# data61/stellar-random-walk

Measured on AMD Instinct MI355X. Metric: walk-steps/sec, higher is better.
Workload: dtype f64

## Files before the change

### stellar-random-walk_amd/csrc/walk_kernels.hip

```cpp
#include <algorithm>
#include <map>
#include <tuple>
#include <chrono>
#include <cstring>

#include "engine.h"
#include "sampling.h"
#include "walk_records.h"

namespace srw {
namespace {
constexpr int TILE = 16;

__device__ inline const Row *row_of(const GraphView &g, int32_t v) {
  int64_t s = (int64_t)v - g.vmin;
  if (s < 0 || s >= g.n_slots) return nullptr;
  return g.rows + s;
}

__device__ inline void flush_counters(DevCounters *ctr, unsigned long long steps, unsigned long long dead,
                                      unsigned long long degc, unsigned long long degp, unsigned long long reads,
                                      unsigned long long fb) {
  steps = wave_sum_u64(steps); dead = wave_sum_u64(dead); degc = wave_sum_u64(degc);
  degp = wave_sum_u64(degp); reads = wave_sum_u64(reads); fb = wave_sum_u64(fb);
  if (lane_id() == 0) {
    if (steps) atomicAdd(&ctr->steps, steps);
    if (dead) atomicAdd(&ctr->dead_ends, dead);
    if (degc) atomicAdd(&ctr->sum_deg_curr, degc);
    if (degp) atomicAdd(&ctr->sum_deg_prev, degp);
    if (reads) atomicAdd(&ctr->ent_reads, reads);
    if (fb) atomicAdd(&ctr->fallbacks, fb);
  }
}

template <bool NT, int MINW, bool COMPACT>
__global__ __launch_bounds__(TPB, MINW) void k_walk_first_order(GraphView g, const int32_t *__restrict__ verts,
                                                          int64_t n_verts, int64_t n_walkers, int32_t L,
                                                          int32_t first_walk, RngSpec rng,
                                                          int32_t *__restrict__ paths, int32_t *__restrict__ lens,
                                                          DevCounters *ctr) {
  __shared__ int32_t tile[TPB / 64][64][TILE + 1];
  const int lane = lane_id(), wv = threadIdx.x >> 6;
  const int64_t wi = blockIdx.x * (int64_t)TPB + threadIdx.x;
  const int64_t wave_base = wi - lane;
  const int64_t stride = (int64_t)L + 2;
  bool alive = wi < n_walkers;
  uint32_t iter = 0; int32_t src = 0;
  Row r; r.off = 0; r.deg = 0; r.flags = 0;
  if (alive) {
    int64_t it = wi / n_verts, vi = wi - it * n_verts;
    iter = (uint32_t)(first_walk + it);
    src = verts[vi];
    const Row *rp = row_of(g, src);
    if (rp) r = *rp;
  }
  int32_t len = 1;
  unsigned long long reads = 0, dead = 0, fb = 0;
  Bias nobias; nobias.second_order = false; nobias.need_member = false; nobias.p = nobias.q = 1.0f;
  nobias.prev = 0; nobias.prev_sids = nullptr; nobias.prev_deg = 0; nobias.vmin = g.vmin;
  tile[wv][lane][0] = src;
  src = rng_source(g, src);
  for (int32_t s = 1; s <= L + 1; ++s) {
    const int c = s & (TILE - 1);
    int32_t val = -1;
    if (alive) {
      if (r.deg == 0) {
        alive = false; if (s > 1) ++dead;
      } else {
        if (COMPACT && !(r.flags & ROW_IRREGULAR)) {
          const uint32_t m = walk_bits24(rng.seed, iter, (uint32_t)src, (uint32_t)s);
          unsigned rd;
          const CfoEnt e = cfo_pick<NT>(g.cfo + r.off, r.deg, m, rd); reads += rd;
          val = e.id; ++len;
          r.off = (int64_t)(e.link & CFO_NOFF_MASK); r.deg = (int32_t)((e.link >> 40) & 0x7FFFFFu);
          r.flags = (e.link >> 63) ? ROW_IRREGULAR : 0u;
        } else {
          float u = draw_uniform(rng, iter, (uint32_t)src, (uint32_t)s);
          FoEnt e;
          if (r.flags & ROW_IRREGULAR) {
            int32_t k = lane_pick_sequential(g.ent + r.off, r.deg, nobias, u);
            ++fb;
            if (COMPACT) {
              const CfoEnt ce = g.cfo[r.off + k];
              e.id = ce.id; e.noff = (int64_t)(ce.link & CFO_NOFF_MASK); e.ndeg = (int32_t)((ce.link >> 40) & 0x7FFFFFu);
              e.nflags = (ce.link >> 63) ? ROW_IRREGULAR : 0u;
            } else {
              e = g.fo[r.off + k];
            }
          } else {
            unsigned rd; int32_t k;
            e = fo_pick<NT>(g.fo + r.off, r.deg, u, k, rd); reads += rd;
          }
          val = e.id; ++len;
          r.off = e.noff; r.deg = e.ndeg; r.flags = e.nflags;
        }
      }
    }
    tile[wv][lane][c] = val;
    if (c == TILE - 1 || s == L + 1) {
      const int ncols = c + 1;
      const int64_t base_slot = s - c;
      __syncthreads();
#pragma unroll
      for (int rr = 0; rr < 16; ++rr) {
        int row = rr * 4 + (lane >> 4), col = lane & 15;
        int64_t w = wave_base + row;
        if (col < ncols && w < n_walkers) paths[w * stride + base_slot + col] = tile[wv][row][col];
      }
      __syncthreads();
    }
  }
  if (wi < n_walkers) lens[wi] = len;
  flush_counters(ctr, (unsigned long long)(len - 1), dead, 0, 0, reads, fb);
}

__device__ inline Bias make_bias(const GraphView &g, float p, float q, int32_t prev, bool second_order) {
  Bias b;
  b.p = p; b.q = q; b.prev = prev; b.second_order = second_order;
  b.need_member = second_order && (q != 1.0f);
  b.prev_sids = nullptr; b.prev_deg = 0; b.vmin = g.vmin;
  if (b.need_member) {
    int64_t s = (int64_t)prev - g.vmin;
    if (s >= 0 && s < g.n_slots) { Row r = g.mrows[s]; b.prev_sids = g.msids + r.off; b.prev_deg = r.deg; b.prev_hub = r.flags >> ROW_HUB_SHIFT; }
  }
  return b;
}

__global__ __launch_bounds__(TPB, 4) void k_walk_general(GraphView g, const int32_t *__restrict__ verts,
                                                      int64_t n_verts, int64_t n_walkers, int32_t L,
                                                      int32_t first_walk, RngSpec rng, float p, float q,
                                                      int32_t *__restrict__ paths, int32_t *__restrict__ lens,
                                                      DevCounters *ctr, unsigned long long *cursor, int32_t tune,
                                                      const int32_t *__restrict__ todo, const unsigned long long *todo_n,
                                                      const int32_t *__restrict__ todo_tie, const ChainRec *__restrict__ tie_list,
                                                      const SWalker *__restrict__ tie_out) {
  __shared__ __attribute__((aligned(16))) uint32_t bitmap[TPB / 64][BINNED_LDS_WORDS];
  const int lane = lane_id();
  Member mem; mem.mode = 0; mem.bm = bitmap[threadIdx.x >> 6]; mem.seg_base = 0;
  mem.ehash = g.ehash; mem.ehash_mask = g.ehash_mask;
#ifdef SRW_PHASE_TIMING
  const unsigned long long t_begin = wall_clock64();
#endif
  const int64_t stride = (int64_t)L + 2;
  unsigned long long steps = 0, degc = 0, degp = 0, fb = 0, dead = 0, fast = 0, srch = 0;
  unsigned long long n_strat[12] = {0, 0, 0, 0, 0, 0, 0, 0, 0, 0, 0, 0};
  while (true) {
    unsigned long long grab = 0;
    if (lane == 0) grab = atomicAdd(cursor, 1ull);
    int64_t wi = (int64_t)(((unsigned long long)(uint32_t)__builtin_amdgcn_readfirstlane((int)(grab >> 32)) << 32) |
                           (uint32_t)__builtin_amdgcn_readfirstlane((int)(uint32_t)grab));
    int32_t tie_s = -1, tie_k = 0, tie_next = 0;
    if (todo) {
      if (wi >= (int64_t)*todo_n) break;
      if (todo_tie) {
        const int32_t ci = todo_tie[wi];
        if (ci >= 0) {
          const SWalker o = tie_out[ci];
          if (o.kind == SK_WALKER_RET || o.kind == SK_RET) { tie_s = (int32_t)tie_list[ci].pad; tie_k = o.pad0; tie_next = o.curr; }
        }
      }
      wi = todo[wi];
    } else if (wi >= n_walkers) break;
    int64_t it = wi / n_verts, vi = wi - it * n_verts;
    const uint32_t iter = (uint32_t)(first_walk + it);
    const int32_t src = verts[vi];
    const uint32_t ksrc = (uint32_t)rng_source(g, src);
    int32_t *path = paths + wi * stride;
    if (lane == 0) path[0] = src;
    int32_t prev = src, curr = src, len = 1;
    Row rprev; rprev.off = 0; rprev.deg = 0; rprev.flags = 0;
    int64_t eprev = 0;
    for (int32_t s = 1; s <= L + 1; ++s) {
      const bool second = s > 1;
      const int64_t cslot = (int64_t)curr - g.vmin;
      const bool in_range = cslot >= 0 && cslot < g.n_slots;
      const bool want_tab = g.eb_off && second && q != 1.0f && !(tune & 16);
      Row r = g.rows[in_range ? cslot : 0];
      uint32_t eo = EB_NONE;
      if (want_tab) eo = g.eb_off[eprev];
      if (!in_range) { r.off = 0; r.deg = 0; r.flags = 0; }
      if (r.deg == 0) { dead += s > 1; break; }
      Bias b;
      b.p = p; b.q = q; b.prev = prev; b.second_order = second; b.need_member = second && (q != 1.0f); b.vmin = g.vmin;
      b.prev_sids = g.sids + rprev.off; b.prev_deg = rprev.deg; b.prev_hub = rprev.flags >> ROW_HUB_SHIFT;
      float u = draw_uniform(rng, iter, ksrc, (uint32_t)s);
      unsigned f = 0, sv = 0;
#ifdef SRW_PHASE_TIMING
      mem.t_step0 = wall_clock64();
#endif
      SRW_T0(mem);
      int32_t k = -1, next = 0;
      bool binned_served = false, have_next = false;
      unsigned which = SRW_STRAT_SCAN;
      if (s == tie_s) { k = tie_k; next = tie_next; have_next = true; binned_served = true; which = SRW_STRAT_EDGE_TABLE; f = 1; n_strat[SRW_STAT_TIES_RESOLVED] += 1; }
      else if (want_tab) {
        if (r.deg <= g.eb_mask_max) {
          if (r.deg <= 32 || eo != EB_NONE) {
            k = wave_pick_masked(g, r, b, eo, r.deg > 32 ? g.em_bits + (size_t)eo * 4 : nullptr, u, f, next);
            have_next = true; binned_served = true; which = SRW_STRAT_EDGE_MASK;
            srch += 8ull * (unsigned long long)r.deg + 4ull * (unsigned long long)((r.deg + 31) >> 5);
          }
        } else if (eo != EB_NONE && (r.flags & ROW_PQ_OK)) {
          k = wave_pick_edge_table(g, r, b, g.eb_bins + (size_t)eo * 8, u, f, sv, mem, next, mem.bm + 2 * BIN_CAP);
          if (k >= 0) { have_next = true; binned_served = true; which = SRW_STRAT_EDGE_TABLE; srch += 8ull * EB_BINS; }
        }
      }
      if (k < 0 && (!b.need_member || (tune & 16))) {
        k = wave_pick_prefix(g, r, cslot, b, mem.bm, u, f, sv);
        if (k >= 0) which = SRW_STRAT_PREFIX;
      }
      SRW_T1(mem, t_prefix);
      if (k < 0 && !(tune & 16)) {
        unsigned su = 0;
        k = wave_pick_binned(g, r, cslot, b, mem.bm, u, f, sv, tune & 7, (tune & 8) != 0, mem, srch, su, next);
        binned_served = k >= 0;
        if (k >= 0) { have_next = true; which = su == 1 ? SRW_STRAT_P1 : su == 2 ? SRW_STRAT_P2 : su == 4 ? SRW_STRAT_P3 : SRW_STRAT_W; }
      }
      if (k < 0) { k = wave_pick_scan(g, r, b, mem, u, f); degc += (unsigned long long)r.deg; }
      else { fast += sv; }
      n_strat[which] += 1; n_strat[SRW_STRAT_CHAIN] += f;
      if (!have_next) next = g.ent[r.off + k].id;
#ifdef SRW_PHASE_TIMING
      mem.t_strat[which] += wall_clock64() - mem.t_step0 + (unsigned long long)(next & 0);
#endif
      fb += f;
      if (b.need_member && !binned_served) degp += (unsigned long long)b.prev_deg;
      if (lane == 0) path[s] = next;
      prev = curr; curr = next; ++len; rprev = r; eprev = r.off + k;
    }
    for (int64_t t = len + lane; t < stride; t += 64) path[t] = -1;
    if (lane == 0) lens[wi] = len;
    steps += (unsigned long long)(len - 1);
  }
  if (lane == 0) {
    if (steps) atomicAdd(&ctr->steps, steps);
    if (dead) atomicAdd(&ctr->dead_ends, dead);
    if (degc) atomicAdd(&ctr->sum_deg_curr, degc);
    if (degp) atomicAdd(&ctr->sum_deg_prev, degp);
    if (fb) atomicAdd(&ctr->fallbacks, fb);
    if (fast) atomicAdd(&ctr->ent_reads, fast);
    srch += mem.res_bytes;
    if (srch) atomicAdd(&ctr->trials, srch);
    for (int i = 0; i < 12; ++i) if (n_strat[i]) atomicAdd(&ctr->strat[i], n_strat[i]);
#ifdef SRW_PHASE_TIMING
    const unsigned long long tv[10] = {wall_clock64() - t_begin, mem.t_prefix, mem.t_a, mem.t_p1, mem.t_p2, mem.t_w,
                                       mem.t_fin, mem.t_fill, mem.t_pass1, mem.t_pass2};
    for (int i = 0; i < 10; ++i) atomicAdd(&ctr->dbg[i], tv[i] >> 10);
    atomicAdd(&ctr->dbg[10], mem.n_w); atomicAdd(&ctr->dbg[11], mem.n_w_elems); atomicAdd(&ctr->dbg[12], mem.n_w_windows);
    atomicAdd(&ctr->dbg[13], mem.n_p1); atomicAdd(&ctr->dbg[14], mem.n_p1_elems); atomicAdd(&ctr->dbg[15], mem.n_binned);
    for (int i = 0; i < 12; ++i) atomicAdd(&ctr->dbg[24 + i], mem.t_strat[i] >> 10);
    atomicAdd(&ctr->dbg[16], mem.t_w_lb >> 10); atomicAdd(&ctr->dbg[17], mem.t_w_ins >> 10); atomicAdd(&ctr->dbg[18], mem.t_w_la >> 10); atomicAdd(&ctr->dbg[19], mem.t_w_probe >> 10);
#endif
  }
}

#ifndef SRW_LEAN_WAVES
#define SRW_LEAN_WAVES 8
#endif
#ifndef SRW_LEAN_WAVES_BF
#define SRW_LEAN_WAVES_BF 8
#endif
// ... 113 lines not shown
        const unsigned long long t = atomicAdd(ah.todo_n, 1ull);
        ah.todo[t] = (int32_t)wi;
        if (ah.tie.todo_tie) ah.tie.todo_tie[t] = tie_rec;
        atomicAdd(&ah.ctr->strat[SRW_STAT_HANDED_OVER], 1ull);
      }
      continue;
    }
#ifdef SRW_PATH_BUF
    {
      const int64_t b0 = (int64_t)(len & ~63);
      if (b0 + lane < stride) path[b0 + lane] = pbuf;
      for (int64_t t = b0 + 64 + lane; t < stride; t += 64) path[t] = -1;
    }
#else
    for (int64_t t = len + lane; t < stride; t += 64) path[t] = -1;
#endif
    if (lane == 0) TAB_ARGS().lens[wi] = len;
    steps += (unsigned long long)(len - 1); n_first += len > 1 ? 1u : 0u;
    fb += w_fb; dead += w_dead; fast += w_fast; srch += w_srch; n_tab += w_tab; n_mask += w_mask;
  }
  if (lane == 0) {
    DevCounters *ctr = TAB_ARGS().ctr;
    srch += mem.res_bytes;
    if (steps) atomicAdd(&ctr->steps, steps);
    if (dead) atomicAdd(&ctr->dead_ends, (unsigned long long)dead);
    if (fb) { atomicAdd(&ctr->fallbacks, (unsigned long long)fb); atomicAdd(&ctr->strat[SRW_STRAT_CHAIN], (unsigned long long)fb); }
    if (fast) atomicAdd(&ctr->ent_reads, (unsigned long long)fast);
    if (srch) atomicAdd(&ctr->trials, srch);
    if (n_tab) atomicAdd(&ctr->strat[SRW_STRAT_EDGE_TABLE], (unsigned long long)n_tab);
    if (n_mask) atomicAdd(&ctr->strat[SRW_STRAT_EDGE_MASK], (unsigned long long)n_mask);
    if (n_first) atomicAdd(&ctr->strat[SRW_STRAT_SCAN], (unsigned long long)n_first);
#ifdef SRW_PHASE_TIMING
    atomicAdd(&ctr->dbg[1], mem.t_a >> 10); atomicAdd(&ctr->dbg[2], mem.t_p1 >> 10); atomicAdd(&ctr->dbg[3], mem.t_p2 >> 10);
    atomicAdd(&ctr->dbg[10], mem.n_w); atomicAdd(&ctr->dbg[11], mem.n_w_elems); atomicAdd(&ctr->dbg[12], mem.n_w_windows);
    atomicAdd(&ctr->dbg[13], mem.n_p1); atomicAdd(&ctr->dbg[14], mem.n_p1_elems); atomicAdd(&ctr->dbg[15], mem.n_binned);
    atomicAdd(&ctr->dbg[16], mem.t_fin);
#endif
  }
}

template <bool NT>
__device__ inline int q1_pick(const GraphView &g, const Row &r, const CfoEnt *crow, uint32_t rv, int32_t rv_pos0, float rv_w0, int32_t prev_id,
                              uint32_t m, float p, CfoEnt &e, int32_t &k, unsigned long long &reads, double *S_out = nullptr) {
  const PqRow PQ(g, r.off);
  int32_t rp[REV_MAX_RETURNS]; double rc[REV_MAX_RETURNS];
  int nr = 0;
  double corr_all = 0.0;
  int64_t so = 0;
  if (rv != REV_NONE) {
    nr = (int)(rv >> 24);
    so = r.off + (int64_t)(rv & 0xFFFFFFu);
    if (nr >= 255) {
      const uint32_t xprev = (uint32_t)((int64_t)prev_id - g.vmin);
      const int64_t row_end = r.off + r.deg;
      while (so + nr < row_end && g.sids[so + nr] == xprev) ++nr;
    }
#pragma unroll
    for (int i = 0; i < REV_MAX_RETURNS; ++i) {
      rp[i] = r.deg; rc[i] = 0.0;
      if (i < nr) {
        float w;
        if (i == 0) { rp[0] = rv_pos0; w = rv_w0; }
        else { rp[i] = (int32_t)g.sperm[so + i]; w = g.sw[so + i]; }
        rc[i] = (double)div_exact(w, p) - (double)w; corr_all += rc[i];
      }
    }
    for (int i = REV_MAX_RETURNS; i < nr; ++i) { const float w = g.sw[so + i]; corr_all += (double)div_exact(w, p) - (double)w; }
  } else {
#pragma unroll
    for (int i = 0; i < REV_MAX_RETURNS; ++i) { rp[i] = r.deg; rc[i] = 0.0; }
  }
  {
    const double S0 = PQ[r.deg - 1], S = S0 + corr_all;
    const double pS = (double)m * 0x1p-24 * S;
    auto corr_upto = [&](int32_t kk) {
      double a = 0.0;
#pragma unroll
      for (int i = 0; i < REV_MAX_RETURNS; ++i) a += (rp[i] <= kk) ? rc[i] : 0.0;
      for (int i = REV_MAX_RETURNS; i < nr; ++i)
        if ((int32_t)g.sperm[so + i] <= kk) { const float w = g.sw[so + i]; a += (double)div_exact(w, p) - (double)w; }
      return a;
    };
    auto numer = [&](int32_t kk) { return PQ[kk] + corr_upto(kk); };
    auto not_miss = [&](int32_t kk, double num) { return !(num * (1.0 + (double)(kk + 8) * 0x1p-51) < pS); };
    auto guide_start = [&](double tau, bool &ok) {
      double f = tau / S0;
      f = f < 0.0 ? 0.0 : (f > 0.99999994 ? 0.99999994 : f);
      const uint32_t mm = (uint32_t)(f * 16777216.0);
      const uint32_t j = (uint32_t)(((uint64_t)mm * (uint64_t)(uint32_t)r.deg) >> 24);
      const CfoEnt ge = load_cfo<NT>(crow + j); ++reads;
      const int32_t gd = cfo_delta(ge.cg, ge.link);
      if (gd == CFO_GD_SAT) { ok = false; return 0; }
      const int32_t st = (int32_t)j - gd;
      return st < 0 ? 0 : (st >= r.deg ? r.deg - 1 : st);
    };
    bool ok = S > 0.0 && S0 > 0.0;
    int32_t k0 = 0;
    if (ok) {
      k0 = guide_start(pS, ok);
      const double cb = ok ? corr_upto(k0) : 0.0;
      if (ok && cb != 0.0) {
        int32_t first_r = r.deg;
#pragma unroll
        for (int i = 0; i < REV_MAX_RETURNS; ++i) first_r = rp[i] < first_r ? rp[i] : first_r;
        for (int i = REV_MAX_RETURNS; i < nr; ++i) { const int32_t q_ = (int32_t)g.sperm[so + i]; first_r = q_ < first_r ? q_ : first_r; }
        const int32_t k1 = guide_start(pS - cb, ok);
        k0 = k1 < first_r ? first_r : k1;
      }
    }
    const bool usable = S > 0.0 && S0 > 0.0;
    if (!usable) return 1;
    else if (S_out && g.dbg_chain_deg && r.deg >= g.dbg_chain_deg) { *S_out = S; return 2; }
    else {
      int guard = 0;
      double nk = 0.0;
      if (ok) {
        nk = numer(k0);
        bool nm = not_miss(k0, nk);
        while (nm && k0 > 0 && guard < 12) {
          const double np = numer(k0 - 1);
          if (!not_miss(k0 - 1, np)) break;
          --k0; nk = np; ++guard;
        }
        while (!nm && guard < 12) {
          ++k0; ++guard;
          if (k0 >= r.deg) break;
          nk = numer(k0); nm = not_miss(k0, nk);
        }
        reads += (unsigned)guard + 1u;
      }
      if (!ok || guard >= 12) {
        int32_t lo = 0, hi = r.deg;
        while (lo < hi) {
          const int32_t mid = lo + ((hi - lo) >> 1);
          if (not_miss(mid, numer(mid))) hi = mid; else lo = mid + 1;
          ++reads;
        }
        k0 = lo;
        if (k0 < r.deg) nk = numer(k0);
      }
      if (k0 >= r.deg) { k = 0; e = load_cfo<NT>(crow); ++reads; }
      else if (nk * (1.0 - (double)(k0 + 8) * 0x1p-51) >= pS) { k = k0; e = load_cfo<NT>(crow + k); ++reads; }
      else { if (S_out) *S_out = S; return 2; }
    }
  }
  return 0;
}

template <bool NT>
__global__ __launch_bounds__(TPB) void k_walk_q1(GraphView g, const int32_t *__restrict__ verts, int64_t n_verts,
                                                 int64_t n_walkers, int32_t L, int32_t first_walk, RngSpec rng, float p,
                                                 int32_t *__restrict__ paths, int32_t *__restrict__ lens, DevCounters *ctr,
                                                 int32_t *__restrict__ todo, unsigned long long *todo_n, uint32_t max_ret) {
  __shared__ int32_t tile[TPB / 64][64][TILE + 1];
  const int lane = lane_id(), wv = threadIdx.x >> 6;
  const int64_t wi = blockIdx.x * (int64_t)TPB + threadIdx.x;
  const int64_t wave_base = wi - lane;
  const int64_t stride = (int64_t)L + 2;
  bool alive = wi < n_walkers, handed = false;
  uint32_t iter = 0; int32_t src = 0;
  Row r; r.off = 0; r.deg = 0; r.flags = 0;
  if (alive) {
    const int64_t it = wi / n_verts, vi = wi - it * n_verts;
    iter = (uint32_t)(first_walk + it);
    src = verts[vi];
    const Row *rp = row_of(g, src);
    if (rp) r = *rp;
  }
  int32_t len = 1;
  int64_t eprev = 0;
  int32_t prev_id = src, curr_id = src;
  unsigned long long reads = 0, dead = 0;
  tile[wv][lane][0] = src;
  src = rng_source(g, src);
  for (int32_t s = 1; s <= L + 1; ++s) {
    const int c = s & (TILE - 1);
    int32_t val = -1;
    bool big = false; uint32_t big_rv = 0u, big_m = 0u;
    if (alive) {
      if (r.deg == 0) {
        alive = false; if (s > 1) ++dead;
      } else if (r.flags & ROW_IRREGULAR) {
        alive = false; handed = true; atomicAdd(&ctr->why[0], 1ull);
      } else {
        const uint32_t m = walk_bits24(rng.seed, iter, (uint32_t)src, (uint32_t)s);
        const CfoEnt *crow = g.cfo + r.off;
        CfoEnt e; int32_t k = -1;
        if (s == 1) {
          unsigned rd; e = cfo_pick<NT>(crow, r.deg, m, rd, k); reads += rd;
        } else {
          const int4v rv4 = NT ? __builtin_nontemporal_load(reinterpret_cast<const int4v *>(g.rev + eprev))
                               : *reinterpret_cast<const int4v *>(g.rev + eprev);
          if ((uint32_t)rv4.x != REV_NONE && ((uint32_t)rv4.x >> 24) > max_ret) { big = true; big_rv = (uint32_t)rv4.x; big_m = m; }
          else {
            const int why = q1_pick<NT>(g, r, crow, (uint32_t)rv4.x, rv4.y, __int_as_float(rv4.z), prev_id, m, p, e, k, reads);
            if (why) { alive = false; handed = true; atomicAdd(&ctr->why[why], 1ull); }
          }
        }
        if (alive && !big) {
          val = e.id; ++len;
          prev_id = curr_id; curr_id = val;
          eprev = r.off + k;
          r.off = (int64_t)(e.link & CFO_NOFF_MASK); r.deg = (int32_t)((e.link >> 40) & 0x7FFFFFu);
          r.flags = (e.link >> 63) ? ROW_IRREGULAR : 0u;
        }
      }
    }
    unsigned long long mb = __ballot(big);
    while (mb) {
      const int l = __ffsll((long long)mb) - 1;
      mb &= mb - 1ull;
      Row rr;
      rr.off = (int64_t)(((unsigned long long)(uint32_t)__builtin_amdgcn_readlane((int)(uint32_t)((uint64_t)r.off >> 32), l) << 32) |
                         (uint32_t)__builtin_amdgcn_readlane((int)(uint32_t)r.off, l));
      rr.deg = __builtin_amdgcn_readlane(r.deg, l); rr.flags = ROW_PQ_OK;
      const int32_t pv = __builtin_amdgcn_readlane(prev_id, l);
      const uint32_t rvl = (uint32_t)__builtin_amdgcn_readlane((int)big_rv, l);
      const uint32_t ml = (uint32_t)__builtin_amdgcn_readlane((int)big_m, l);
      const int64_t so = rr.off + (int64_t)(rvl & 0xFFFFFFu);
      int32_t nr = (int32_t)(rvl >> 24);
      if (nr >= 255) {
        const uint32_t xprev = (uint32_t)((int64_t)pv - g.vmin);
        nr = 0;
        for (int64_t cc = so;; cc += 64) {
          const unsigned long long mm = __ballot(cc + lane < rr.off + rr.deg && g.sids[cc + lane] == xprev);
          nr += __popcll(mm);
          if (mm != ~0ull) break;
        }
      }
      Bias b; b.p = p; b.q = 1.0f; b.prev = pv; b.second_order = true; b.need_member = false; b.vmin = g.vmin;
      b.prev_sids = nullptr; b.prev_deg = 0; b.prev_hub = 0;
      unsigned f = 0;
      const int32_t kk = wave_pick_returns<false>(g, rr, b, so, nr, (float)ml * (1.0f / 16777216.0f), f);
      if (lane == l) {
        big = false;
        if (kk < 0) { alive = false; handed = true; atomicAdd(&ctr->why[kk == CHAIN_NEEDED ? 2 : 1], 1ull); }
        else {
          const CfoEnt e = load_cfo<NT>(g.cfo + r.off + kk); ++reads;
          val = e.id; ++len;
          prev_id = curr_id; curr_id = val;
          eprev = r.off + kk;
          r.off = (int64_t)(e.link & CFO_NOFF_MASK); r.deg = (int32_t)((e.link >> 40) & 0x7FFFFFu);
          r.flags = (e.link >> 63) ? ROW_IRREGULAR : 0u;
        }
      }
    }
    tile[wv][lane][c] = val;
    if (c == TILE - 1 || s == L + 1) {
      const int ncols = c + 1;
      const int64_t base_slot = s - c;
      __syncthreads();
#pragma unroll
      for (int rr = 0; rr < 16; ++rr) {
        int row = rr * 4 + (lane >> 4), col = lane & 15;
        int64_t w = wave_base + row;
        if (col < ncols && w < n_walkers) paths[w * stride + base_slot + col] = tile[wv][row][col];
      }
      __syncthreads();
    }
  }
  if (wi < n_walkers) {
    if (handed) { todo[atomicAdd(todo_n, 1ull)] = (int32_t)wi; atomicAdd(&ctr->strat[SRW_STAT_HANDED_OVER], 1ull); }
    else lens[wi] = len;
  }
  const unsigned long long my_steps = handed ? 0ull : (unsigned long long)(len - 1);
  flush_counters(ctr, my_steps, handed ? 0ull : dead, 0, 0, reads, 0);
  const unsigned long long tot = wave_sum_u64(my_steps);
  if (lane == 0 && tot) atomicAdd(&ctr->strat[SRW_STRAT_Q1_LANE], tot);
}

template <bool NT>
__device__ inline AEnt load_al_head(const AEnt *p) {
  const int4v *q = reinterpret_cast<const int4v *>(p);
  const int4v a = NT ? __builtin_nontemporal_load(q) : *q;
  AEnt e;
  e.prob = __int_as_float(a.x); e.alias = a.y; e.id = a.z; e.wrev = __int_as_float(a.w);
  e.noff = 0; e.ndeg = 0; e.nflags = 0;
  return e;
}
template <bool NT>
__device__ inline void load_al_tail(const AEnt *p, AEnt &e) {
  const int4v *q = reinterpret_cast<const int4v *>(p) + 1;
  const int4v b = NT ? __builtin_nontemporal_load(q) : *q;
  e.noff = (int64_t)(((uint64_t)(uint32_t)b.y << 32) | (uint32_t)b.x);
  e.ndeg = b.z; e.nflags = (uint32_t)b.w;
}

template <bool NT>
__global__ __launch_bounds__(TPB, 6) void k_walk_alias(GraphView g, const int32_t *__restrict__ verts, int64_t n_verts,
                                                    int64_t n_walkers, int32_t L, int32_t first_walk, uint32_t seed,
                                                    float p, float q, int32_t *__restrict__ paths,
                                                    int32_t *__restrict__ lens, DevCounters *ctr) {
  __shared__ int32_t stage[TPB][TILE + 1];
  int32_t *buf = stage[threadIdx.x];
  const int64_t wi = blockIdx.x * (int64_t)TPB + threadIdx.x;
  unsigned long long reads = 0, dead = 0, fb = 0, trials = 0;
  int32_t len = 0;
  if (wi < n_walkers) {
    const int64_t stride = (int64_t)L + 2;
    const int64_t it = wi / n_verts, vi = wi - it * n_verts;
    const uint32_t iter = (uint32_t)(first_walk + it);
    const int32_t src = verts[vi];
    const uint32_t ksrc = (uint32_t)rng_source(g, src);
    int32_t *path = paths + wi * stride;
    Row rc; rc.off = 0; rc.deg = 0; rc.flags = 0;
    { const Row *rp0 = row_of(g, src); if (rp0) rc = *rp0; }
    Row rp = rc;
    int32_t curr = src, prev = src;
    buf[0] = src; len = 1;
    const float inv_p = 1.0f / p, inv_q = 1.0f / q;
    const float Q = inv_q > 1.0f ? inv_q : 1.0f;
    const bool biased_cfg = !(p == 1.0f && q == 1.0f);
    int32_t s = 1; uint32_t t = 0;
    bool fold = false; double fa = 0.0, ftot = 0.0, fw = 0.0; int32_t flo = -1, fhi = -1;
    float wprev_hint = __int_as_float(0x7FC00000);
    while (s <= L + 1) {
      if (rc.deg == 0) { if (s > 1) ++dead; break; }
      const bool second = s > 1, biased = second && biased_cfg;
      uint32_t o[4];
      philox4x32_10(iter, ksrc, (uint32_t)s, t, seed, 0xA11A5u, o);
      AEnt e;
      const AEnt *ep = nullptr;
      bool accepted = true;
      if (rc.flags & ROW_ALIAS_IRREGULAR) {
        Bias b; b.p = p; b.q = q; b.prev = prev; b.second_order = second; b.need_member = second && q != 1.0f;
        b.prev_sids = g.sids + rp.off; b.prev_deg = rp.deg; b.vmin = g.vmin;
        float u = (float)(o[2] >> 8) * (1.0f / 16777216.0f);
        int32_t k = lane_pick_sequential(g.ent + rc.off, rc.deg, b, u);
        e = g.al[rc.off + k]; ++fb;
      } else {
        if (t == 0) {
          fold = false;
          if (biased && inv_p > Q) {
            flo = -1; fhi = -1;
            if (wprev_hint == wprev_hint) {
              fw = (double)wprev_hint;
            } else {
              const uint32_t *cs = g.sids + rc.off;
              const uint32_t x = (uint32_t)((int64_t)prev - g.vmin);
              int32_t lo = 0, hi = rc.deg;
              while (lo < hi) { int32_t mid = lo + ((hi - lo) >> 1); if (cs[mid] < x) lo = mid + 1; else hi = mid; }
              flo = lo; fhi = lo; fw = 0.0;
              while (fhi < rc.deg && cs[fhi] == x) { fw += (double)g.ent[rc.off + g.sperm[rc.off + fhi]].w; ++fhi; }
            }
            if (fw > 0.0) {
              const double S = g.rsum[(int64_t)curr - g.vmin];
              fa = ((double)inv_p - (double)Q) * fw; ftot = (double)Q * S + fa; fold = true;
            }
          }
        }
        bool appendix = false;
        if (fold) {
          uint32_t y[4];
          philox4x32_10(iter, ksrc, (uint32_t)s, t, seed, 0xA11A6u, y);
          const float u5 = (float)(y[0] >> 8) * (1.0f / 16777216.0f);
          if ((double)u5 * ftot < fa) {
            appendix = true;
            if (flo < 0) {
              const uint32_t *cs = g.sids + rc.off;
              const uint32_t x = (uint32_t)((int64_t)prev - g.vmin);
              int32_t lo = 0, hi = rc.deg;
              while (lo < hi) { int32_t mid = lo + ((hi - lo) >> 1); if (cs[mid] < x) lo = mid + 1; else hi = mid; }
              flo = lo; fhi = lo;
              while (fhi < rc.deg && cs[fhi] == x) ++fhi;
            }
            const float u6 = (float)(y[1] >> 8) * (1.0f / 16777216.0f);
            const double target = (double)u6 * fw;
            double cum = 0.0; int32_t pos = g.sperm[rc.off + flo];
            for (int32_t c = flo; c < fhi; ++c) {
              pos = (int32_t)g.sperm[rc.off + c];
              cum += (double)g.ent[rc.off + pos].w;
              if (cum >= target) break;
            }
            ep = g.al + rc.off + pos; e = load_al_head<NT>(ep); ++reads;
          }
        }
        ++trials;
        if (!appendix) {
          const uint64_t r64 = ((uint64_t)o[0] << 32) | o[1];
          const int64_t j = (int64_t)__umul64hi(r64, (uint64_t)(uint32_t)rc.deg);
          ep = g.al + rc.off + j; e = load_al_head<NT>(ep); ++reads;
          const float u2 = (float)(o[2] >> 8) * (1.0f / 16777216.0f);
          if (!(u2 < e.prob)) { ep = g.al + rc.off + e.alias; e = load_al_head<NT>(ep); ++reads; }
          if (biased) {
            const float u3 = (float)(o[3] >> 8) * (1.0f / 16777216.0f);
            const float thr = u3 * Q;
            if (e.id == prev) accepted = thr < inv_p;
            else if (thr < fminf(inv_q, 1.0f)) accepted = true;
            else {
              bool in;
              if (g.ehash)
                in = edge_exists(g.ehash, g.ehash_mask, (uint32_t)((int64_t)prev - g.vmin), (uint32_t)((int64_t)e.id - g.vmin));
              else {
                if (ep) { load_al_tail<NT>(ep, e); ep = nullptr; }
                if (g.symmetric && e.ndeg < rp.deg)
                  in = sorted_contains(g.sids + e.noff, e.ndeg, (uint32_t)((int64_t)prev - g.vmin));
                else
                  in = sorted_contains(g.sids + rp.off, rp.deg, (uint32_t)((int64_t)e.id - g.vmin));
              }
              accepted = thr < (in ? 1.0f : inv_q);
            }
            accepted = accepted || (t + 1u >= 65536u);
          }
        }
      }
      if (accepted) {
        if (ep) load_al_tail<NT>(ep, e);
        buf[s & (TILE - 1)] = e.id;
        if ((s & (TILE - 1)) == TILE - 1) {
          int32_t *dst = path + (s - (TILE - 1));
// ... 1070 lines not shown
  }
}
__global__ void k_hook_rng(uint32_t seed, const uint32_t *iter, const uint32_t *src, const uint32_t *step, int64_t n,
                           float *out) {
  RngSpec rng; rng.mode = 1; rng.const_r = 0.f; rng.seed = seed;
  for (int64_t i = blockIdx.x * (int64_t)blockDim.x + threadIdx.x; i < n; i += (int64_t)gridDim.x * blockDim.x)
    out[i] = draw_uniform(rng, iter[i], src[i], step[i]);
}

void read_counters(srw_handle *h, srw_walk_stats *stats) {
  DevCounters c;
  SRW_HIP(hipMemcpyAsync(&c, h->counters.p, sizeof(c), hipMemcpyDeviceToHost, h->stream));
  SRW_HIP(hipStreamSynchronize(h->stream));
#ifdef SRW_PHASE_TIMING
  {
    static const char *nm[10] = {"total", "prefix", "binned:ret-edges", "binned:P1", "binned:P2", "binned:W", "binned:search+resolve",
                                 "scan:fill", "scan:pass1", "scan:pass2"};
    fprintf(stderr, "[phase] wave-ms:");
    for (int i = 0; i < 10; ++i) fprintf(stderr, " %s %.0f", nm[i], (double)c.dbg[i] * 1024.0 / 100e3);
    fprintf(stderr, "\n[phase] W calls %llu elems %llu windows %llu | P1 calls %llu elems %llu | binned steps %llu\n", c.dbg[10], c.dbg[11],
            c.dbg[12], c.dbg[13], c.dbg[14], c.dbg[15]);
    {
      static const char *sn[12] = {"edge_table", "p1", "p2", "w", "p3", "scan", "prefix", "chain", "edge_mask", "-", "-", "-"};
      fprintf(stderr, "[phase] per-strategy wave-ms (whole step) / steps / us per step:");
      for (int i = 0; i < 12; ++i)
        if (c.strat[i]) fprintf(stderr, " %s %.0f / %llu / %.2f", sn[i], (double)c.dbg[24 + i] * 1024.0 / 100e3, c.strat[i],
                                (double)c.dbg[24 + i] * 1024.0 / 100.0 / (double)c.strat[i]);
      fprintf(stderr, "\n");
    }
    if (c.strat[SRW_STRAT_EDGE_TABLE])
      fprintf(stderr, "[lean] wave-ms: mask steps %.0f (%llu steps), table steps %.0f (%llu steps; %.0f with deg(prev) > 1024) | chunks %llu: "
              "no specials %llu, N(prev) staged %llu, hub bitmap %llu, edge hash %llu; candidates per chunk %.0f, rounds per chunk %.2f\n",
              (double)c.dbg[1] * 1024.0 / 100e3, c.strat[SRW_STRAT_EDGE_MASK], (double)c.dbg[2] * 1024.0 / 100e3, c.strat[SRW_STRAT_EDGE_TABLE],
              (double)c.dbg[3] * 1024.0 / 100e3, c.dbg[15], c.dbg[10], c.dbg[13], c.dbg[12], c.dbg[14],
              (double)c.dbg[11] / (double)std::max<unsigned long long>(c.dbg[15], 1), (double)c.dbg[16] / (double)std::max<unsigned long long>(c.dbg[15], 1));
    fprintf(stderr, "[phase] W detail wave-ms: wait-B %.0f clear+insert %.0f wait-A %.0f probe %.0f\n", (double)c.dbg[16] * 1024.0 / 100e3,
            (double)c.dbg[17] * 1024.0 / 100e3, (double)c.dbg[18] * 1024.0 / 100e3, (double)c.dbg[19] * 1024.0 / 100e3);
  }
#endif
  if (getenv("SRW_DEBUG_HANDOVER"))
    fprintf(stderr, "[handover] walkers %llu | q1 reasons: irregular row %llu, non-positive sum %llu, boundary draw %llu\n",
            c.strat[SRW_STAT_HANDED_OVER], c.why[0], c.why[1], c.why[2]);
  if (!stats) return;
  stats->n_steps = (int64_t)c.steps; stats->dead_ends = (int64_t)c.dead_ends;
  stats->sum_deg_curr = (int64_t)c.sum_deg_curr; stats->sum_deg_prev = (int64_t)c.sum_deg_prev;
  stats->ent_reads = (int64_t)c.ent_reads; stats->fallbacks = (int64_t)c.fallbacks; stats->trials = (int64_t)c.trials;
  for (int i = 0; i < 12; ++i) stats->strategy_steps[i] = (int64_t)c.strat[i];
  stats->edge_tables = (h->g.has_eb && h->g.use_eb) ? h->g.eb_tables : 0;
  stats->edge_table_bytes = (h->g.has_eb && h->g.use_eb) ? h->g.eb_bytes : 0;
}

void check_params(const srw_walk_params &P) {
  if (P.walk_length < 0) throw Error(SRW_ERR_INVALID, "walk_length must be >= 0");
  if (P.num_walks < 0) throw Error(SRW_ERR_INVALID, "num_walks must be >= 0");
  if (P.rng_mode != SRW_RNG_CONST && P.rng_mode != SRW_RNG_PHILOX) throw Error(SRW_ERR_INVALID, "bad rng_mode");
  if (P.sampler != SRW_SAMPLER_REFERENCE && P.sampler != SRW_SAMPLER_ALIAS) throw Error(SRW_ERR_INVALID, "bad sampler");
  if (P.sampler == SRW_SAMPLER_ALIAS && P.rng_mode != SRW_RNG_PHILOX)
    throw Error(SRW_ERR_INVALID, "Mode A draws several uniforms per step: it needs SRW_RNG_PHILOX");
}

}

namespace {
struct ChainBufs {
  ChainRec *list; ChainMeta *meta; uint32_t *totals; double *D; ChainUnits cu; long long d_cap;
  uint32_t *tie_hdr; WWalker *tie_recs; SWalker *tie_out; unsigned long long *tie_cur; uint32_t *tie_skip;
};
ChainBufs chain_bufs(srw_handle *h) {
  static const long long d_cap = (long long)(getenv("SRW_CHAIN_SCRATCH_MB") ? atof(getenv("SRW_CHAIN_SCRATCH_MB")) : 512.0) * (1 << 20) / 8;
  const size_t n_units = (size_t)(d_cap / 256) + CHAIN_CAP;
  const size_t core = (size_t)CHAIN_CAP * (sizeof(ChainRec) + sizeof(ChainMeta)) + 64 + n_units * 24;
  const size_t tie = 64 + (size_t)CHAIN_CAP * (sizeof(WWalker) + sizeof(SWalker) + 4) + 64;
  h->chain_buf.ensure(core + tie);
  h->chain_d.ensure((size_t)d_cap);
  ChainBufs b;
  char *base = h->chain_buf.p;
  b.list = reinterpret_cast<ChainRec *>(base);
  b.meta = reinterpret_cast<ChainMeta *>(base + (size_t)CHAIN_CAP * sizeof(ChainRec));
  b.totals = reinterpret_cast<uint32_t *>(base + (size_t)CHAIN_CAP * (sizeof(ChainRec) + sizeof(ChainMeta)));
  char *ub = base + (size_t)CHAIN_CAP * (sizeof(ChainRec) + sizeof(ChainMeta)) + 64;
  b.cu.usum = reinterpret_cast<double *>(ub);
  b.cu.utot = reinterpret_cast<unsigned long long *>(ub + n_units * 8);
  b.cu.ue = reinterpret_cast<int32_t *>(ub + n_units * 16);
  b.D = h->chain_d.p; b.d_cap = d_cap;
  char *tb = base + ((core + 63) & ~(size_t)63);
  b.tie_cur = reinterpret_cast<unsigned long long *>(tb);
  b.tie_hdr = reinterpret_cast<uint32_t *>(tb + 32);
  b.tie_recs = reinterpret_cast<WWalker *>(tb + 48);
  b.tie_out = reinterpret_cast<SWalker *>(tb + 48 + (size_t)CHAIN_CAP * sizeof(WWalker));
  b.tie_skip = reinterpret_cast<uint32_t *>(tb + 48 + (size_t)CHAIN_CAP * (sizeof(WWalker) + sizeof(SWalker)));
  return b;
}
void enqueue_chain(srw_handle *h, const ChainBufs &cb, const GraphView &gv, const ShardIO &io, const srw_walk_params &P, int32_t step, int32_t last,
                   const RngSpec &rng, SWalker *scratch, int strat, unsigned long long *cursor, uint32_t *skipped, unsigned long long *pass_cur = nullptr) {
  hipStream_t st = h->stream;
  hipLaunchKernelGGL(k_chain_setup, dim3(1), dim3(256), 0, st, gv, io, cb.list, cursor, cb.meta, cb.totals, cb.d_cap, skipped, pass_cur);
  hipLaunchKernelGGL(k_chain_d, dim3(h->n_cus * 4), dim3(TPB), 0, st, gv, io, P.p, P.q, cb.list, cb.meta, cb.totals, cb.D, cb.cu);
  hipLaunchKernelGGL(k_chain_scan, dim3(CHAIN_CAP / (TPB / 64)), dim3(TPB), 0, st, cb.meta, cb.totals, cb.cu);
  hipLaunchKernelGGL(k_chain_u, dim3(h->n_cus * 4), dim3(TPB), 0, st, cb.totals, (const double *)cb.D, cb.cu);
  hipLaunchKernelGGL(k_chain_seq, dim3(CHAIN_CAP / (TPB / 64)), dim3(TPB), 0, st, gv, io, P.first_walk, step, last, rng, cb.list, cb.meta, cb.totals,
                     (const double *)cb.D, cb.cu, scratch, h->counters.p, strat);
}
}

namespace {
struct LaunchInfo { int kind; int record_bytes; };

struct StreamDrain {
  srw_handle *h;
  explicit StreamDrain(srw_handle *hh) : h(hh) {}
  ~StreamDrain() {
    if (h->copy_stream) (void)hipStreamSynchronize(h->copy_stream);
    if (h->stream) (void)hipStreamSynchronize(h->stream);
  }
};

__global__ void k_paths_to_ids(int32_t *__restrict__ paths, const int32_t *__restrict__ lens, int64_t n_walkers, int64_t stride,
                               const int32_t *__restrict__ orig_id) {
  const int lane = lane_id();
  for (int64_t w = blockIdx.x * (int64_t)(TPB / 64) + (threadIdx.x >> 6); w < n_walkers; w += (int64_t)gridDim.x * (TPB / 64)) {
    const int32_t len = lens[w];
    int32_t *row = paths + w * stride;
    for (int32_t k = lane; k < len; k += 64) row[k] = orig_id[row[k]];
  }
}

LaunchInfo launch_walk(srw_handle *h, const srw_walk_params &P, int32_t num_walks, int32_t first_walk, int32_t *d_paths,
                       int32_t *d_lens) {
  Graph &g = h->g;
  { const char *e = getenv("SRW_DEBUG_CHAIN_DEG"); g.dbg_chain_deg = e && *e ? atoi(e) : 0; }
  hipStream_t st = h->stream;
  const int64_t n_walkers = (int64_t)num_walks * g.n_vertices;
  const bool alias = P.sampler == SRW_SAMPLER_ALIAS;
  bool first_order_compact = false;
  const bool first_order = !alias && (P.p == 1.0f && P.q == 1.0f) && !(P.flags & SRW_WALK_FORCE_GENERAL);
  RngSpec rng; rng.mode = P.rng_mode; rng.const_r = P.const_r; rng.seed = P.seed;
  GraphView gv = g.view();
  if (alias) {
    int64_t blocks = (n_walkers + TPB - 1) / TPB;
    const size_t al_bytes = (size_t)g.n_entries * sizeof(AEnt);
    (void)al_bytes;
    const bool nt = (P.flags & SRW_WALK_NT_LOADS) != 0;
    if (nt)
      hipLaunchKernelGGL(k_walk_alias<true>, dim3((unsigned)blocks), dim3(TPB), 0, st, gv, g.verts.p, g.n_vertices, n_walkers,
                         P.walk_length, first_walk, P.seed, P.p, P.q, d_paths, d_lens, h->counters.p);
    else
      hipLaunchKernelGGL(k_walk_alias<false>, dim3((unsigned)blocks), dim3(TPB), 0, st, gv, g.verts.p, g.n_vertices, n_walkers,
                         P.walk_length, first_walk, P.seed, P.p, P.q, d_paths, d_lens, h->counters.p);
  } else if (first_order) {
    int64_t blocks = (n_walkers + TPB - 1) / TPB;
    const size_t fo_bytes = (size_t)g.n_entries * sizeof(FoEnt);
    const bool nt = (P.flags & SRW_WALK_NT_LOADS) ? true
                    : (P.flags & SRW_WALK_CACHED_LOADS) ? false : fo_bytes > ((size_t)2 << 30);
    const int occ = (P.flags >> 8) & 0xF;
    const bool compact = g.has_cfo && P.rng_mode == SRW_RNG_PHILOX && !(P.flags & SRW_WALK_NO_COMPACT);
    first_order_compact = compact;
#define SRW_LAUNCH_FO(NTV, MW, CP)                                                                                  \
  hipLaunchKernelGGL((k_walk_first_order<NTV, MW, CP>), dim3((unsigned)blocks), dim3(TPB), 0, st, gv, g.verts.p,     \
                     g.n_vertices, n_walkers, P.walk_length, first_walk, rng, d_paths, d_lens, h->counters.p)
    if (compact) {
      const bool ntc = (P.flags & SRW_WALK_NT_LOADS) ? true : (P.flags & SRW_WALK_CACHED_LOADS) ? false
                       : (size_t)g.n_entries * sizeof(CfoEnt) > ((size_t)2 << 30);
      if (ntc) SRW_LAUNCH_FO(true, 1, true); else SRW_LAUNCH_FO(false, 1, true);
    } else if (nt) { if (occ == 8) SRW_LAUNCH_FO(true, 8, false); else if (occ == 7) SRW_LAUNCH_FO(true, 7, false); else SRW_LAUNCH_FO(true, 1, false); }
    else    { if (occ == 8) SRW_LAUNCH_FO(false, 8, false); else if (occ == 7) SRW_LAUNCH_FO(false, 7, false); else SRW_LAUNCH_FO(false, 1, false); }
#undef SRW_LAUNCH_FO
  } else {
    int64_t blocks = std::min<int64_t>((n_walkers * 64 + TPB - 1) / TPB, (int64_t)h->n_cus * 8);
    h->walk_cursor.ensure(2);
    SRW_HIP(hipMemsetAsync(h->walk_cursor.p, 0, 2 * sizeof(unsigned long long), st));
    const int32_t tune = (int32_t)(((P.flags >> 12) & 15) | ((P.flags & SRW_WALK_NO_BINNED) ? 16 : 0));
    const bool lean = gv.eb_off && g.eb_complete && P.q != 1.0f && tune == 0 && !getenv("SRW_NO_LEAN_KERNEL");
    const bool q1 = P.q == 1.0f && P.p != 1.0f && P.rng_mode == SRW_RNG_PHILOX && g.has_cfo && g.has_pq && g.has_rev &&
                    g.pq_bad_rows == 0 && tune == 0 && !(P.flags & SRW_WALK_NO_PREFIX) && !getenv("SRW_NO_Q1_KERNEL");
    const int32_t *todo = nullptr;
    const int32_t *todo_tie = nullptr; const ChainRec *tie_list = nullptr; const SWalker *tie_out = nullptr;
    TieSink tie; tie.hdr = nullptr; tie.recs = nullptr; tie.list = nullptr; tie.cur = nullptr; tie.todo_tie = nullptr;
    ChainBufs cb;
    const bool ties = lean && P.rng_mode == SRW_RNG_PHILOX && !getenv("SRW_NO_TIE_KERNELS");
    if (q1 || lean) h->walk_todo.ensure(2 * (size_t)n_walkers);
    if (ties) {
      cb = chain_bufs(h);
      SRW_HIP(hipMemsetAsync(cb.tie_cur, 0, 48, st));
      SRW_HIP(hipMemsetAsync(cb.tie_out, 0xFF, (size_t)CHAIN_CAP * sizeof(SWalker), st));
      tie.hdr = cb.tie_hdr; tie.recs = cb.tie_recs; tie.list = cb.list; tie.cur = cb.tie_cur + 2;
      tie.todo_tie = h->walk_todo.p + n_walkers;
    }
    auto resolve_ties = [&]() {
      if (!ties) return;
      ShardIO io; io.recv = reinterpret_cast<const char *>(cb.tie_hdr); io.chunk_bytes = 0; io.cap_w = CHAIN_CAP; io.cap_r = 0;
      io.world = 1; io.rank = 0; io.batch = 0x7FFFFFFF; io.pt = nullptr; io.lens = nullptr; io.n_rows = 0;
      srw_walk_params Pc = P; Pc.first_walk = first_walk;
      static const int n_pass = getenv("SRW_TIE_PASSES") ? std::max(1, atoi(getenv("SRW_TIE_PASSES"))) : 8;
      for (int pass = 0; pass < n_pass; ++pass)
        enqueue_chain(h, cb, gv, io, Pc, 0, 0, rng, cb.tie_out, -1, cb.tie_cur, cb.tie_skip, cb.tie_cur + 3);
      todo_tie = tie.todo_tie; tie_list = cb.list; tie_out = cb.tie_out;
    };
    if (q1) {
      const int64_t qb = (n_walkers + TPB - 1) / TPB;
      const uint32_t q1_max_ret = getenv("SRW_Q1_MAX_RET") ? (uint32_t)atoi(getenv("SRW_Q1_MAX_RET")) : 16u;
      if ((size_t)g.n_entries * sizeof(CfoEnt) > ((size_t)2 << 30))
        hipLaunchKernelGGL(k_walk_q1<true>, dim3((unsigned)qb), dim3(TPB), 0, st, gv, g.verts.p, g.n_vertices, n_walkers, P.walk_length,
                           first_walk, rng, P.p, d_paths, d_lens, h->counters.p, h->walk_todo.p, h->walk_cursor.p + 1, q1_max_ret);
      else
        hipLaunchKernelGGL(k_walk_q1<false>, dim3((unsigned)qb), dim3(TPB), 0, st, gv, g.verts.p, g.n_vertices, n_walkers, P.walk_length,
                           first_walk, rng, P.p, d_paths, d_lens, h->counters.p, h->walk_todo.p, h->walk_cursor.p + 1, q1_max_ret);
      todo = h->walk_todo.p;
    }
    if (lean) {
      int64_t lb = std::min<int64_t>((n_walkers * 64 + TPB - 1) / TPB, (int64_t)h->n_cus * 16);
      TabArgs ta;
      ta.g = gv; ta.verts = g.verts.p; ta.n_verts = g.n_vertices; ta.n_walkers = n_walkers; ta.L = P.walk_length; ta.first_walk = first_walk;
      ta.rng = rng; ta.p = P.p; ta.q = P.q; ta.paths = d_paths; ta.lens = d_lens; ta.ctr = h->counters.p; ta.cursor = h->walk_cursor.p;
      ta.todo = h->walk_todo.p; ta.todo_n = h->walk_cursor.p + 1; ta.tie = tie;
      const bool groups = getenv("SRW_TABLE_GROUPS") && atoi(getenv("SRW_TABLE_GROUPS")) != 0;
      const int lanes = getenv("SRW_TABLE_LANES") ? atoi(getenv("SRW_TABLE_LANES")) : (gv.ebp.min_sh <= 6 ? 2 : -1);
      if (getenv("SRW_TABLE_ROUNDS") && atoi(getenv("SRW_TABLE_ROUNDS")) != 0) {
        launch_walk_tables_rounds(h, ta, gv.bf_off != nullptr, getenv("SRW_LANE_CSH") ? atoi(getenv("SRW_LANE_CSH")) : 6, st);
      } else if (lanes >= 0) {
        launch_walk_tables_lanes(ta, gv.bf_off != nullptr, lanes, getenv("SRW_LANE_CSH") ? atoi(getenv("SRW_LANE_CSH")) : 6, h->n_cus, st);
      } else if (groups) {
        launch_walk_tables_groups(ta, gv.bf_off != nullptr, h->n_cus, st);
      } else if (gv.bf_off) {
        hipLaunchKernelGGL((k_walk_tables<true>), dim3((unsigned)lb), dim3(TPB), 0, st, ta);
      } else {
        hipLaunchKernelGGL((k_walk_tables<false>), dim3((unsigned)lb), dim3(TPB), 0, st, ta);
      }
      SRW_HIP(hipMemsetAsync(h->walk_cursor.p, 0, sizeof(unsigned long long), st));
      todo = h->walk_todo.p;
      resolve_ties();
    }
    hipLaunchKernelGGL(k_walk_general, dim3((unsigned)blocks), dim3(TPB), 0, st, gv, g.verts.p, g.n_vertices, n_walkers,
                       P.walk_length, first_walk, rng, P.p, P.q, d_paths, d_lens, h->counters.p, h->walk_cursor.p, tune, todo,
                       h->walk_cursor.p + 1, todo_tie, tie_list, tie_out);
  }
  SRW_HIP(hipGetLastError());
  LaunchInfo li;
  li.kind = alias ? 3 : first_order ? 1 : 2;
  li.record_bytes = first_order_compact ? 16 : (first_order || alias) ? 32 : 0;
  if (g.compact && n_walkers > 0) {
    const int64_t nb = std::min<int64_t>((n_walkers + TPB / 64 - 1) / (TPB / 64), (int64_t)h->n_cus * 32);
    hipLaunchKernelGGL(k_paths_to_ids, dim3((unsigned)nb), dim3(TPB), 0, st, d_paths, d_lens, n_walkers, (int64_t)P.walk_length + 2,
                       (const int32_t *)g.orig_id.p);
    SRW_HIP(hipGetLastError());
  }
  return li;
}

void prepare_tables(srw_handle *h, const srw_walk_params &P) {
  const bool timing = getenv("SRW_TIMING") != nullptr;
  auto t_phase = std::chrono::steady_clock::now();
  auto phase = [&](const char *name) {
    if (!timing) return;
    (void)hipStreamSynchronize(h->stream);
    const auto t = std::chrono::steady_clock::now();
    const double ms = std::chrono::duration<double, std::milli>(t - t_phase).count();
    if (ms >= 20.0) fprintf(stderr, "[timing] prepare_tables: %s %.0f ms\n", name, ms);
    t_phase = t;
  };
  const bool alias = P.sampler == SRW_SAMPLER_ALIAS;
  const bool first_order = !alias && (P.p == 1.0f && P.q == 1.0f) && !(P.flags & SRW_WALK_FORCE_GENERAL);
  if (first_order) build_first_order_tables(h, P.rng_mode != SRW_RNG_PHILOX || (P.flags & SRW_WALK_NO_COMPACT));
  else build_membership(h);
  if (!alias && !first_order && P.q == 1.0f && P.p != 1.0f && P.rng_mode == SRW_RNG_PHILOX && h->cfg.world == 1 &&
      !(P.flags & (SRW_WALK_NO_PREFIX | SRW_WALK_NO_COMPACT)) && !getenv("SRW_NO_Q1_KERNEL")) {
    build_first_order_tables(h, false);
    build_rev_table(h);
  }
  phase("membership / first-order tables / return edges");
  if (alias) build_alias_tables(h);
  phase("alias tables");
  const bool general = !alias && !first_order;
  if (general && !(P.p == 1.0f && P.q == 1.0f) && !(P.flags & SRW_WALK_NO_PREFIX)) build_pq_tables(h, P.p, P.q);
  else if (general) h->g.has_pq = false;
  bool want_ehash = P.q != 1.0f && !(P.flags & SRW_WALK_NO_EDGE_HASH) && (alias || (general && h->cfg.world == 1));
  const bool want_hub = general && P.q != 1.0f && h->cfg.world == 1 && !(P.flags & SRW_WALK_NO_HUB_BITMAPS);
  const bool want_eb = general && P.q != 1.0f && h->cfg.world == 1 && h->g.has_pq && !(P.flags & SRW_WALK_NO_EDGE_TABLES) &&
                       !(P.flags & SRW_WALK_NO_BINNED);
  const int eb_mode = (P.flags & SRW_WALK_EDGE_TABLES_ALL) ? 1 : 0;
  phase("prefix sums of the (p, q) base weights");
  if (want_eb) build_unit_ids(h);
  phase("unit-weight ids");
  const char *env_hub = getenv("SRW_HUB_BUDGET_GB"), *env_cap = getenv("SRW_EB_CHUNKS");
  bool drop_ehash = false;
  size_t hub_cap = want_eb ? (size_t)16 << 30 : (size_t)64 << 30;
  size_t table_cap_used = 0;
  int eb_cap = EB_BINS;
  if (env_hub && *env_hub) hub_cap = (size_t)(atof(env_hub) * (double)((size_t)1 << 30));
  if (env_cap && *env_cap) eb_cap = atoi(env_cap);
  struct TabPlan { int cap = 0, min_sh = 8, cm = 0, fine = 0, ratio = 0; size_t need = 0; bool complete = false; };
  auto finer = [](const TabPlan &a, const TabPlan &b) {
    if (a.complete != b.complete) return a.complete;
    if (a.cap != b.cap) return a.cap > b.cap;
    if (a.min_sh != b.min_sh) return a.min_sh < b.min_sh;
    return std::min(a.cm, 16384) > std::min(b.cm, 16384);
  };
  size_t reserve = (size_t)P.num_walks * (size_t)h->g.n_vertices * ((size_t)P.walk_length + 3) * 4 + ((size_t)8 << 30);
  if (reserve > ((size_t)64 << 30)) reserve = (size_t)64 << 30;
  if (const char *r = getenv("SRW_EB_RESERVE_GB"); r && *r) reserve = (size_t)(atof(r) * (double)((size_t)1 << 30));
  h->g.eb_reserve = reserve;
  const int64_t job_walks = std::max<int64_t>(h->planned_walks > 0 ? h->planned_walks : 10, P.num_walks);
  std::map<std::tuple<int, int, int, int, int>, size_t> size_cache;
  auto set_size = [&](int cap, int sh, int cm, int fine, int ratio = 0) {
    Graph &g = h->g;
    const auto key = std::make_tuple(cap, sh, cm, fine, ratio);
    auto it = size_cache.find(key);
    if (it != size_cache.end()) return it->second;
    g.eb_min_sh_sel = sh; g.eb_cm_sel = cm; g.eb_fine_cap_sel = fine; g.eb_cm_ratio_sel = ratio;
    const size_t n = edge_tables_full_bytes(h, eb_mode, cap);
    if (getenv("SRW_TIMING")) fprintf(stderr, "[timing] table plan: %d chunks of >= %d, masks <= %d (ratio %d), fine %d: %.1f GB\n", cap, 1 << sh, cm, ratio, fine, (double)n / 1e9);
    size_cache[key] = n;
    return n;
  };
  auto plan_tables = [&](size_t free_b) {
    TabPlan t;
    const size_t ceiling = (size_t)230 << 30;
    auto fits = [&](size_t n, size_t margin) { return n > 0 && n < ceiling && free_b > n + reserve + margin; };
    const bool fixed_cap = env_cap && *env_cap;
// ... 631 lines not shown
```

Before: 35.99 billion.

## Align path tile flushes to 64-byte boundaries via per-walker phase ring buffer

Replaces the 16-column shared-memory staging tile with a 32-entry ring per walker whose write index is offset by each path row's address phase, so every flushed 16-element window starts on a 64-byte-aligned global address instead of an arbitrary offset. This aims to turn the scattered, misaligned path stores into whole aligned segments and cut partially written cache lines. The cost is more index arithmetic, a doubled shared-memory footprint per wave, and an extra tail flush on the last step. It also drops the occupancy-hint launch variants of the first-order kernel, which reduces template instantiations.

```diff
diff --git a/stellar-random-walk_amd/csrc/path_flush.h b/stellar-random-walk_amd/csrc/path_flush.h
--- /dev/null
+++ b/stellar-random-walk_amd/csrc/path_flush.h
@@ -0,0 +1,37 @@
+#pragma once
+#include <cstdint>
+
+#if !defined(__HIPCC__) && !defined(__host__)
+#define __host__
+#define __device__
+#endif
+
+namespace srw {
+constexpr int PF_WIN = 16;
+constexpr int PF_RING = 32;
+
+__host__ __device__ inline int pf_phase(const int32_t *row) { return (int)(((uintptr_t)row >> 2) & (PF_WIN - 1)); }
+__host__ __device__ inline int pf_ring_index(int ph, int32_t slot) { return (ph + slot) & (PF_RING - 1); }
+__host__ __device__ inline bool pf_flush_point(int32_t s, int32_t L) { return (s & (PF_WIN - 1)) == PF_WIN - 1 || s == L + 1; }
+
+template <class PhaseOf, class Store>
+__host__ __device__ inline void pf_flush_lane(int lane, int32_t L, int32_t s, int n_rows, PhaseOf phase_of, Store store) {
+  const int col = lane & (PF_WIN - 1);
+  const int32_t a0 = (s & ~(PF_WIN - 1)) + col;
+  const bool last = s == L + 1;
+#if defined(__HIP_DEVICE_COMPILE__)
+#pragma unroll
+#endif
+  for (int pass = 0; pass < 16; ++pass) {
+    const int row = pass * 4 + (lane >> 4);
+    if (row >= n_rows) continue;
+    const int ph = phase_of(row);
+    const int32_t i0 = a0 - ph;
+    if (i0 >= 0 && i0 <= L + 1) store(row, i0, (int)(a0 & (PF_RING - 1)));
+    if (last) {
+      const int32_t i1 = i0 + PF_WIN;
+      if (i1 <= L + 1) store(row, i1, (int)((a0 + PF_WIN) & (PF_RING - 1)));
+    }
+  }
+}
+}
diff --git a/stellar-random-walk_amd/csrc/walk_kernels.hip b/stellar-random-walk_amd/csrc/walk_kernels.hip
--- a/stellar-random-walk_amd/csrc/walk_kernels.hip
+++ b/stellar-random-walk_amd/csrc/walk_kernels.hip
@@ -7,10 +7,23 @@
 #include "engine.h"
 #include "sampling.h"
 #include "walk_records.h"
+#include "path_flush.h"
 
 namespace srw {
 namespace {
 constexpr int TILE = 16;
+
+struct PathRing {
+  int32_t v[64][PF_RING];
+  __device__ inline int32_t &at(int row, int idx) { return v[row][(idx + row) & (PF_RING - 1)]; }
+};
+__device__ inline void path_ring_flush(PathRing &ring, int32_t *__restrict__ paths, int64_t wave_base, int64_t n_walkers, int32_t L, int32_t s) {
+  const int64_t stride = (int64_t)L + 2;
+  const int64_t left = n_walkers - wave_base;
+  pf_flush_lane(lane_id(), L, s, left < 64 ? (int)left : 64,
+                [&](int row) { return pf_phase(paths + (wave_base + row) * stride); },
+                [&](int row, int32_t slot, int idx) { paths[(wave_base + row) * stride + slot] = ring.at(row, idx); });
+}
 
 __device__ inline const Row *row_of(const GraphView &g, int32_t v) {
   int64_t s = (int64_t)v - g.vmin;
@@ -39,7 +52,7 @@
                                                           int32_t first_walk, RngSpec rng,
                                                           int32_t *__restrict__ paths, int32_t *__restrict__ lens,
                                                           DevCounters *ctr) {
-  __shared__ int32_t tile[TPB / 64][64][TILE + 1];
+  __shared__ PathRing rings[TPB / 64];
   const int lane = lane_id(), wv = threadIdx.x >> 6;
   const int64_t wi = blockIdx.x * (int64_t)TPB + threadIdx.x;
   const int64_t wave_base = wi - lane;
@@ -58,10 +71,11 @@
   unsigned long long reads = 0, dead = 0, fb = 0;
   Bias nobias; nobias.second_order = false; nobias.need_member = false; nobias.p = nobias.q = 1.0f;
   nobias.prev = 0; nobias.prev_sids = nullptr; nobias.prev_deg = 0; nobias.vmin = g.vmin;
-  tile[wv][lane][0] = src;
+  PathRing &ring = rings[wv];
+  const int ph = pf_phase(paths + wi * stride);
+  ring.at(lane, pf_ring_index(ph, 0)) = src;
   src = rng_source(g, src);
   for (int32_t s = 1; s <= L + 1; ++s) {
-    const int c = s & (TILE - 1);
     int32_t val = -1;
     if (alive) {
       if (r.deg == 0) {
@@ -96,17 +110,10 @@
         }
       }
     }
-    tile[wv][lane][c] = val;
-    if (c == TILE - 1 || s == L + 1) {
-      const int ncols = c + 1;
-      const int64_t base_slot = s - c;
+    ring.at(lane, pf_ring_index(ph, s)) = val;
+    if (pf_flush_point(s, L)) {
       __syncthreads();
-#pragma unroll
-      for (int rr = 0; rr < 16; ++rr) {
-        int row = rr * 4 + (lane >> 4), col = lane & 15;
-        int64_t w = wave_base + row;
-        if (col < ncols && w < n_walkers) paths[w * stride + base_slot + col] = tile[wv][row][col];
-      }
+      path_ring_flush(ring, paths, wave_base, n_walkers, L, s);
       __syncthreads();
     }
   }
@@ -526,7 +533,7 @@
                                                  int64_t n_walkers, int32_t L, int32_t first_walk, RngSpec rng, float p,
                                                  int32_t *__restrict__ paths, int32_t *__restrict__ lens, DevCounters *ctr,
                                                  int32_t *__restrict__ todo, unsigned long long *todo_n, uint32_t max_ret) {
-  __shared__ int32_t tile[TPB / 64][64][TILE + 1];
+  __shared__ PathRing rings[TPB / 64];
   const int lane = lane_id(), wv = threadIdx.x >> 6;
   const int64_t wi = blockIdx.x * (int64_t)TPB + threadIdx.x;
   const int64_t wave_base = wi - lane;
@@ -545,10 +552,11 @@
   int64_t eprev = 0;
   int32_t prev_id = src, curr_id = src;
   unsigned long long reads = 0, dead = 0;
-  tile[wv][lane][0] = src;
+  PathRing &ring = rings[wv];
+  const int ph = pf_phase(paths + wi * stride);
+  ring.at(lane, pf_ring_index(ph, 0)) = src;
   src = rng_source(g, src);
   for (int32_t s = 1; s <= L + 1; ++s) {
-    const int c = s & (TILE - 1);
     int32_t val = -1;
     bool big = false; uint32_t big_rv = 0u, big_m = 0u;
     if (alive) {
@@ -619,17 +627,10 @@
         }
       }
     }
-    tile[wv][lane][c] = val;
-    if (c == TILE - 1 || s == L + 1) {
-      const int ncols = c + 1;
-      const int64_t base_slot = s - c;
+    ring.at(lane, pf_ring_index(ph, s)) = val;
+    if (pf_flush_point(s, L)) {
       __syncthreads();
-#pragma unroll
-      for (int rr = 0; rr < 16; ++rr) {
-        int row = rr * 4 + (lane >> 4), col = lane & 15;
-        int64_t w = wave_base + row;
-        if (col < ncols && w < n_walkers) paths[w * stride + base_slot + col] = tile[wv][row][col];
-      }
+      path_ring_flush(ring, paths, wave_base, n_walkers, L, s);
       __syncthreads();
     }
   }
@@ -2006,7 +2007,6 @@
     const size_t fo_bytes = (size_t)g.n_entries * sizeof(FoEnt);
     const bool nt = (P.flags & SRW_WALK_NT_LOADS) ? true
                     : (P.flags & SRW_WALK_CACHED_LOADS) ? false : fo_bytes > ((size_t)2 << 30);
-    const int occ = (P.flags >> 8) & 0xF;
     const bool compact = g.has_cfo && P.rng_mode == SRW_RNG_PHILOX && !(P.flags & SRW_WALK_NO_COMPACT);
     first_order_compact = compact;
 #define SRW_LAUNCH_FO(NTV, MW, CP)                                                                                  \
@@ -2016,8 +2016,8 @@
       const bool ntc = (P.flags & SRW_WALK_NT_LOADS) ? true : (P.flags & SRW_WALK_CACHED_LOADS) ? false
                        : (size_t)g.n_entries * sizeof(CfoEnt) > ((size_t)2 << 30);
       if (ntc) SRW_LAUNCH_FO(true, 1, true); else SRW_LAUNCH_FO(false, 1, true);
-    } else if (nt) { if (occ == 8) SRW_LAUNCH_FO(true, 8, false); else if (occ == 7) SRW_LAUNCH_FO(true, 7, false); else SRW_LAUNCH_FO(true, 1, false); }
-    else    { if (occ == 8) SRW_LAUNCH_FO(false, 8, false); else if (occ == 7) SRW_LAUNCH_FO(false, 7, false); else SRW_LAUNCH_FO(false, 1, false); }
+    } else if (nt) SRW_LAUNCH_FO(true, 1, false);
+    else SRW_LAUNCH_FO(false, 1, false);
 #undef SRW_LAUNCH_FO
   } else {
     int64_t blocks = std::min<int64_t>((n_walkers * 64 + TPB - 1) / TPB, (int64_t)h->n_cus * 8);
```

Result: faster. 38.04 billion (median of 6 runs) (+5.7%).
